# cadia-lvl/ss_asr

Measured on AMD Instinct MI355X. Metric: train-step utterances/sec on 80-dim mel, higher is better.
Workload: dtype f32; 1 GPU; BASELINE.json configs[1]: one ASRTrainer.exec iteration (GPU batch assembly from the HBM-resident corpus + engine.ASRTrainStep), ~10h synthetic Malromur-shape fbanks (8000 utts, <=800 frames, 80-dim), batch 32 per GPU, bucketed by length, LAS 256/256/128, tf_rate 0.9, Adadelta; global_batch=32, max_frames=800, parallelism=dp1, matrix_products=fp32 as 6 bf16 MFMAs on exact 3-way operand split, fp32 accumulate

## Files before the change

ss_asr_amd/csrc/common.h:

```cpp
#pragma once
#include <hip/hip_runtime.h>
#include <stdint.h>

typedef float f32x4 __attribute__((ext_vector_type(4)));

#define SSASR_OK 0
#define SSASR_EARG (-1)

#define SSASR_LAUNCH_CHECK()                         \
  do {                                               \
    hipError_t e__ = hipGetLastError();              \
    if (e__ != hipSuccess) return (int)e__;          \
  } while (0)

#define SSASR_HIP(call)                              \
  do {                                               \
    hipError_t e__ = (call);                         \
    if (e__ != hipSuccess) return (int)e__;          \
  } while (0)

struct RowMap {
  int64_t ld;
  int64_t inner;
  int64_t so;
// ... 70 lines not shown
__device__ __forceinline__ float half_max(float v) {
  v = fmaxf(v, dpp_move<0xB1>(v));
  v = fmaxf(v, dpp_move<0x4E>(v));
  v = fmaxf(v, dpp_move<0x141>(v));
  v = fmaxf(v, dpp_move<0x140>(v));
  float a;
  const float b = swap16_other(v, a);
  return fmaxf(a, b);
}
__device__ __forceinline__ float wave_sum(float v) {
  v = half_sum(v);
  const auto r = __builtin_amdgcn_permlane32_swap(__float_as_uint(v), __float_as_uint(v), false, false);
  return __uint_as_float(r[0]) + __uint_as_float(r[1]);
}
__device__ __forceinline__ float wave_max(float v) {
  v = half_max(v);
  const auto r = __builtin_amdgcn_permlane32_swap(__float_as_uint(v), __float_as_uint(v), false, false);
  return fmaxf(__uint_as_float(r[0]), __uint_as_float(r[1]));
}

struct GemmDesc {
  const float* A;
  const float* B;
  float* C;
  RowMap ma, mb, mc;
  int M, N, K;
  int ta;
  int tb;
  const float* bias1;
  const float* bias2;
  int act;
  float alpha, beta;
  int splitk;
  int batch;
  int64_t sa, sb, sc, sbias;
  int nseg;
  struct Seg {
    const float* A[2];
    const float* B[2];
    float* C[2];
    RowMap mb;
    int64_t ldc;
    int N, K;
  } seg[2];
  float* colsum[2];
  float* colsum2[2];
  int kcat;
  int64_t ska, skb;
  int tile;
};
int ssasr_launch_gemm(const GemmDesc& g, hipStream_t st);
int ssasr_launch_transpose(const float* src, float* dst, int rows, int cols, hipStream_t st);
int ssasr_launch_bptt_persistent(const float* whhT, float* gates, const float* cs, const float* dy, int64_t ys_s,
                                 int64_t ys_n, const int32_t* lens, float* gx, int32_t* sync_ws, int64_t S,
                                 int64_t N, int64_t H, int dirs, hipStream_t st, int64_t i0 = 0, int64_t i1 = 0,
                                 float* dc_state = nullptr, const float* whh_f = nullptr, const float* whh_r = nullptr,
                                 bool armed = false, const float* tsave = nullptr, void* stop_event = nullptr,
                                 const void* progress = nullptr);
struct SsasrOptions {
  int no_persistent;
  int no_fused_input;
  int bptt_halves_off;
  int bptt_reserve_kb;
  int no_persistent_decoder;
  int no_persistent_decoder_bwd;
  int delay_fwd, delay_bwd, delay_bwd_ksplit;
  int gemm_tile;
  int gemm_trace_lo, gemm_trace_hi;
  int gemm_wide;
  int gemm_bf16;
  int gemm_x6;
  int gemm_kcat;
  int no_windows;
  int bptt_one_launch;
  int wgrad_fused;
  int last_seg_pct;
  int tail_inline;
  int no_residency_check;
  int test_drop_tile;
  int test_drop_attn_slice;
  int test_drop_dec_slice;
  int attn_rph;
  int no_tsave;
};
const SsasrOptions& ssasr_options();
int64_t ssasr_resident_capacity(const void* kernel, int threads, size_t dyn_lds);
size_t ssasr_gemm_min_lds_bytes();
size_t ssasr_lds_reservation_against_gemm(const void* kernel);
bool ssasr_bptt_ksplit_ok(int64_t S, int64_t N, int64_t H, int dirs);
extern "C" int64_t ssasr_bilstm_bwd_gx_floats(int64_t S, int64_t N, int64_t H);
int ssasr_launch_colsum(const float* m, int64_t rows, int cols, int64_t ld, float* out, hipStream_t st,
                        float* out2 = nullptr);
```

ss_asr_amd/csrc/options.hip:

```cpp
#include <cstdlib>
#include <cstring>
#include <map>
#include <mutex>
#include <tuple>
#include "../../include/ssasr.h"
#include "common.h"

namespace {

SsasrOptions g_opt;
std::once_flag g_opt_once;

int env_int(const char* name, int dflt) {
  const char* v = getenv(name);
  return v ? atoi(v) : dflt;
}
int env_flag(const char* name) { return getenv(name) != nullptr; }

void init_options() {
  g_opt.no_persistent = env_flag("SSASR_NO_PERSISTENT");
  g_opt.no_fused_input = env_flag("SSASR_NO_FUSED_INPUT");
  g_opt.bptt_halves_off = env_flag("SSASR_BPTT_HALVES_OFF");
  g_opt.bptt_reserve_kb = env_flag("SSASR_BPTT_SHARED_CU") ? 0 : env_int("SSASR_BPTT_RESERVE_KB", 118);
  g_opt.no_persistent_decoder = env_flag("SSASR_NO_PERSISTENT_DECODER");
  g_opt.no_persistent_decoder_bwd = env_flag("SSASR_NO_PERSISTENT_DECODER_BWD");
  g_opt.delay_fwd = env_int("SSASR_PERSIST_DELAY_FWD", -1);
  g_opt.delay_bwd = env_int("SSASR_PERSIST_DELAY_BWD", -1);
  g_opt.delay_bwd_ksplit = g_opt.delay_bwd;
  g_opt.gemm_tile = env_int("SSASR_GEMM_TILE", 0);
  g_opt.gemm_x6 = env_int("SSASR_GEMM_X6", 1);
  g_opt.gemm_wide = env_int("SSASR_GEMM_WIDE", 1);
  g_opt.gemm_bf16 = env_int("SSASR_GEMM_BF16", 0);
  g_opt.gemm_trace_lo = g_opt.gemm_trace_hi = 0;
  g_opt.gemm_kcat = env_int("SSASR_GEMM_KCAT", 1);
  g_opt.wgrad_fused = env_int("SSASR_WGRAD_FUSED", 1);
  g_opt.bptt_one_launch = env_int("SSASR_BPTT_ONE_LAUNCH", 1);
  g_opt.no_windows = env_flag("SSASR_NO_WINDOWS");
  g_opt.last_seg_pct = env_int("SSASR_LAST_SEG_PCT", 60);
  g_opt.tail_inline = env_int("SSASR_TAIL_INLINE", 1);
  g_opt.no_residency_check = env_flag("SSASR_NO_RESIDENCY_CHECK");
  g_opt.test_drop_tile = env_int("SSASR_TEST_DROP_TILE", -1);
  g_opt.test_drop_attn_slice = env_int("SSASR_TEST_DROP_ATTN_SLICE", -1);
  g_opt.test_drop_dec_slice = env_int("SSASR_TEST_DROP_DEC_SLICE", -1);
  g_opt.attn_rph = env_int("SSASR_ATTN_RPH", 0);
  if (g_opt.attn_rph != 2 && g_opt.attn_rph != 3 && g_opt.attn_rph != 4 && g_opt.attn_rph != 6) g_opt.attn_rph = 0;
  g_opt.no_tsave = env_flag("SSASR_NO_TSAVE");
}

struct Named { const char* name; int SsasrOptions::*field; };
const Named kNames[] = {
    {"SSASR_NO_PERSISTENT", &SsasrOptions::no_persistent},
    {"SSASR_NO_FUSED_INPUT", &SsasrOptions::no_fused_input},
    {"SSASR_BPTT_HALVES_OFF", &SsasrOptions::bptt_halves_off},
    {"SSASR_BPTT_RESERVE_KB", &SsasrOptions::bptt_reserve_kb},
    {"SSASR_NO_PERSISTENT_DECODER", &SsasrOptions::no_persistent_decoder},
    {"SSASR_NO_PERSISTENT_DECODER_BWD", &SsasrOptions::no_persistent_decoder_bwd},
    {"SSASR_PERSIST_DELAY_FWD", &SsasrOptions::delay_fwd},
    {"SSASR_PERSIST_DELAY_BWD", &SsasrOptions::delay_bwd},
    {"SSASR_GEMM_TILE", &SsasrOptions::gemm_tile},
    {"SSASR_GEMM_TRACE_LO", &SsasrOptions::gemm_trace_lo},
    {"SSASR_GEMM_TRACE_HI", &SsasrOptions::gemm_trace_hi},
    {"SSASR_GEMM_X6", &SsasrOptions::gemm_x6},
    {"SSASR_GEMM_WIDE", &SsasrOptions::gemm_wide},
    {"SSASR_GEMM_BF16", &SsasrOptions::gemm_bf16},
    {"SSASR_GEMM_KCAT", &SsasrOptions::gemm_kcat},
    {"SSASR_WGRAD_FUSED", &SsasrOptions::wgrad_fused},
    {"SSASR_BPTT_ONE_LAUNCH", &SsasrOptions::bptt_one_launch},
    {"SSASR_NO_WINDOWS", &SsasrOptions::no_windows},
    {"SSASR_LAST_SEG_PCT", &SsasrOptions::last_seg_pct},
    {"SSASR_TAIL_INLINE", &SsasrOptions::tail_inline},
    {"SSASR_NO_RESIDENCY_CHECK", &SsasrOptions::no_residency_check},
    {"SSASR_TEST_DROP_TILE", &SsasrOptions::test_drop_tile},
    {"SSASR_TEST_DROP_ATTN_SLICE", &SsasrOptions::test_drop_attn_slice},
    {"SSASR_TEST_DROP_DEC_SLICE", &SsasrOptions::test_drop_dec_slice},
    {"SSASR_ATTN_RPH", &SsasrOptions::attn_rph},
    {"SSASR_NO_TSAVE", &SsasrOptions::no_tsave},
};

}

const SsasrOptions& ssasr_options() {
  std::call_once(g_opt_once, init_options);
  return g_opt;
}

extern "C" int ssasr_set_option(const char* name, int value) {
  if (!name) return SSASR_EARG;
  std::call_once(g_opt_once, init_options);
  for (const Named& n : kNames)
    if (strcmp(n.name, name) == 0) {
      g_opt.*(n.field) = value;
      if (n.field == &SsasrOptions::delay_bwd) g_opt.delay_bwd_ksplit = value;
      return SSASR_OK;
    }
  return SSASR_EARG;
}

extern "C" int ssasr_get_option(const char* name, int* value) {
  if (!name || !value) return SSASR_EARG;
  std::call_once(g_opt_once, init_options);
  for (const Named& n : kNames)
    if (strcmp(n.name, name) == 0) { *value = g_opt.*(n.field); return SSASR_OK; }
  return SSASR_EARG;
}

size_t ssasr_lds_reservation_against_gemm(const void* kernel) {
  constexpr size_t CU_LDS = 160 * 1024;
  hipFuncAttributes fa{};
  if (hipFuncGetAttributes(&fa, kernel) != hipSuccess) return 0;
  const size_t own = fa.sharedSizeBytes, gemm = ssasr_gemm_min_lds_bytes();
  if (own + gemm > CU_LDS) return 0;
  return CU_LDS - own - gemm + 1024;
}

int64_t ssasr_resident_capacity(const void* kernel, int threads, size_t dyn_lds) {
  static std::mutex mu;
  static std::map<std::tuple<const void*, int, size_t, int>, int64_t> cache;
  int dev = 0;
  if (hipGetDevice(&dev) != hipSuccess) return 0;
  std::lock_guard<std::mutex> lock(mu);
  const auto key = std::make_tuple(kernel, threads, dyn_lds, dev);
  auto it = cache.find(key);
  if (it != cache.end()) return it->second;
  int per_cu = 0, cus = 0;
  if (hipOccupancyMaxActiveBlocksPerMultiprocessor(&per_cu, kernel, threads, dyn_lds) != hipSuccess) per_cu = 0;
  if (hipDeviceGetAttribute(&cus, hipDeviceAttributeMultiprocessorCount, dev) != hipSuccess) cus = 0;
  const int64_t cap = (int64_t)per_cu * cus;
  cache[key] = cap;
  return cap;
}
```

ss_asr_amd/csrc/rnn.hip:

```cpp
#include <cstdlib>
#include <hip/hip_ext.h>
#include "../../include/ssasr.h"
#include "rnn_kernels.h"

constexpr int SSASR_MAX_SEGMENTS = 8;

int ssasr_launch_transpose(const float* src, float* dst, int rows, int cols, hipStream_t st) {
  dim3 grid((cols + 31) / 32, (rows + 31) / 32), block(32, 8);
  hipLaunchKernelGGL(transpose_kernel, grid, block, 0, st, src, dst, rows, cols);
  SSASR_LAUNCH_CHECK();
  return SSASR_OK;
}

int ssasr_launch_colsum(const float* m, int64_t rows, int cols, int64_t ld, float* out, hipStream_t st,
                        float* out2) {
  if (rows <= 0 || cols <= 0) return SSASR_OK;
  int64_t gy64 = (rows + 255) / 256;
  int gy = gy64 > 64 ? 64 : (int)gy64;
  if (gy < 1) gy = 1;
  dim3 grid((cols + 63) / 64, gy), block(256);
  if (cols % 4 == 0 && ld % 4 == 0 && aligned16(m))
    hipLaunchKernelGGL(colsum4_kernel, grid, block, 0, st, m, rows, cols, ld, out, out2);
  else
    hipLaunchKernelGGL(colsum_kernel, grid, block, 0, st, m, rows, cols, ld, out, out2);
  SSASR_LAUNCH_CHECK();
  return SSASR_OK;
}

static int persist_delay(int opt, int dflt) {
  if (opt < 0) return dflt;
  return opt > 96 ? 96 : opt;
}

static bool grid_fits(const void* kernel, int threads, size_t dyn_lds, int64_t workgroups) {
  if (ssasr_options().no_residency_check) return true;
  const int64_t cap = ssasr_resident_capacity(kernel, threads, dyn_lds);
  return cap <= 0 || workgroups <= cap;
}

constexpr int64_t PERSIST_WINDOW = 128;
static int64_t window_count(int64_t N) { return (N + PERSIST_WINDOW - 1) / PERSIST_WINDOW; }
static int64_t window_width(int64_t N, int64_t w) { return std::min<int64_t>(PERSIST_WINDOW, N - w * PERSIST_WINDOW); }

static const void* fwd_fn(int kpw, int nb, bool fuse) {
#define SSASR_FN(K, NBT) reinterpret_cast<const void*>(lstm_enc_fwd_persistent_kernel<K, NBT>)
  if (fuse) return nb == 1 ? reinterpret_cast<const void*>(lstm_enc_fwd_persistent_kernel<4, 1, 5>)
                           : reinterpret_cast<const void*>(lstm_enc_fwd_persistent_kernel<4, 2, 5>);
  return nb == 1 ? (kpw == 1 ? SSASR_FN(1, 1) : kpw == 2 ? SSASR_FN(2, 1) : kpw == 4 ? SSASR_FN(4, 1) : SSASR_FN(8, 1))
                 : (kpw == 1 ? SSASR_FN(1, 2) : kpw == 2 ? SSASR_FN(2, 2) : kpw == 4 ? SSASR_FN(4, 2) : SSASR_FN(8, 2));
#undef SSASR_FN
}
static void fwd_launch(int kpw, int nb, bool fuse, dim3 grid, hipStream_t st, const EncPersist& p) {
  const dim3 block(FWD_THREADS);
#define SSASR_L(K, NBT) hipLaunchKernelGGL((lstm_enc_fwd_persistent_kernel<K, NBT>), grid, block, 0, st, p)
  if (fuse && nb == 1) hipLaunchKernelGGL((lstm_enc_fwd_persistent_kernel<4, 1, 5>), grid, block, 0, st, p);
  else if (fuse) hipLaunchKernelGGL((lstm_enc_fwd_persistent_kernel<4, 2, 5>), grid, block, 0, st, p);
  else if (nb == 1) { if (kpw == 1) SSASR_L(1, 1); else if (kpw == 2) SSASR_L(2, 1); else if (kpw == 4) SSASR_L(4, 1); else SSASR_L(8, 1); }
  else { if (kpw == 1) SSASR_L(1, 2); else if (kpw == 2) SSASR_L(2, 2); else if (kpw == 4) SSASR_L(4, 2); else SSASR_L(8, 2); }
#undef SSASR_L
}
static int fwd_nb(int64_t Nw, int64_t H) { return (H / 4) * 2 * ((Nw + 15) / 16) <= 256 ? 1 : 2; }
static int64_t fwd_hx_floats_window(int64_t S, int64_t Nw, int64_t H) { return 2 * S * (H / 4) * ((Nw + 7) & ~(int64_t)7) * 4; }

extern "C" int64_t ssasr_bilstm_fwd_hx_floats(int64_t S, int64_t N, int64_t H) {
  if (S <= 0 || N <= 0 || H <= 0 || H % 64 != 0 || (ssasr_options().no_windows && N > PERSIST_WINDOW)) return 0;
  int64_t total = 0;
  for (int64_t w = 0; w < window_count(N); ++w) total += fwd_hx_floats_window(S, window_width(N, w), H);
  return total;
}

extern "C" int ssasr_bilstm_fwd(const float* x, int64_t xs_s, int64_t xs_n, int64_t S, int64_t N,
                                int64_t I, int64_t H, const int32_t* lens,
                                const float* w_ih_f, const float* w_hh_f, const float* b_ih_f,
                                const float* b_hh_f, const float* w_ih_r, const float* w_hh_r,
                                const float* b_ih_r, const float* b_hh_r, float* y, int64_t ys_s,
                                int64_t ys_n, float* gates, float* cs, float* hs, float* hx,
                                int32_t* sync_ws, int armed, float* tsave, void* stream) {
  const SsasrOptions& opt = ssasr_options();
  if (S <= 0 || N <= 0 || I <= 0 || H <= 0 || H % 16 != 0) return SSASR_EARG;
  if (!x || !y || !gates || (!cs && !tsave) || !hs) return SSASR_EARG;
  if (tsave && !aligned16(tsave)) return SSASR_EARG;
  hipStream_t st = (hipStream_t)stream;
  const int64_t rows = S * N;
  const float* wih[2] = {w_ih_f, w_ih_r};
  const float* whh[2] = {w_hh_f, w_hh_r};
  const float* bih[2] = {b_ih_f, b_ih_r};
  const float* bhh[2] = {b_hh_f, b_hh_r};

  auto input_projection = [&]() -> int {
    const bool paired = bih[0] && bhh[0] && bih[1] && bhh[1] && (wih[1] - wih[0]) % 4 == 0 &&
                        (bih[1] - bih[0]) == (bhh[1] - bhh[0]);
    for (int d = 0; d < (paired ? 1 : 2); ++d) {
      GemmDesc g{};
      g.A = x; g.ma = RowMap{0, N, xs_s, xs_n};
      g.B = wih[d]; g.mb = rm_dense(I);
      g.C = gates + d * rows * 4 * H; g.mc = rm_dense(4 * H);
      g.M = (int)rows; g.N = (int)(4 * H); g.K = (int)I;
      g.ta = 0; g.tb = 0; g.bias1 = bih[d]; g.bias2 = bhh[d];
      g.alpha = 1.f; g.beta = 0.f; g.splitk = 1; g.batch = 1;
      if (paired) {
        g.batch = 2; g.sa = 0; g.sb = wih[1] - wih[0]; g.sc = rows * 4 * H; g.sbias = bih[1] - bih[0];
      }
      int rc = ssasr_launch_gemm(g, st);
      if (rc) return rc;
    }
    return SSASR_OK;
  };

  if (ys_s >= (1ll << 31) || ys_n >= (1ll << 31) || rows * 4 * H >= (1ll << 40)) return SSASR_EARG;
  if (!aligned16(w_hh_f) || !aligned16(w_hh_r) || !aligned16(hs)) return SSASR_EARG;
  {
    const int kpw = (int)(H / 64);
    const int64_t nwin = window_count(N);
    bool fits = hx && sync_ws && H % 64 == 0 && (kpw == 1 || kpw == 2 || kpw == 4 || kpw == 8) &&
                aligned16(hx) && aligned16(gates) && aligned16(cs) && aligned16(y) && ys_s % 4 == 0 &&
                ys_n % 4 == 0 && !opt.no_persistent && !(opt.no_windows && nwin > 1);
    bool fuse_in = fits && kpw == 4 && I == 80 && bih[0] && bhh[0] && bih[1] && bhh[1] &&
                   aligned16(x) && aligned16(w_ih_f) && aligned16(w_ih_r) && xs_s % 4 == 0 && xs_n % 4 == 0 &&
                   !opt.no_fused_input;
    for (int64_t w = 0; w < nwin && fits; ++w) {
      const int64_t Nw = window_width(N, w), Npw = (Nw + 7) & ~(int64_t)7;
      const int nb = fwd_nb(Nw, H);
      const int64_t chunks = (Nw + 16 * nb - 1) / (16 * nb);
      if ((H / 4) * 2 * chunks > 512 || S * Npw * H * 4 >= (1ll << 31) ||
          !grid_fits(fwd_fn(kpw, nb, fuse_in), FWD_THREADS, 0, (H / 4) * 2 * chunks)) {
        fits = false; fuse_in = false;
      }
    }
    if (tsave && !fits) return SSASR_EARG;
    if (!fuse_in) {
      const int rc = input_projection();
      if (rc) return rc;
    }
    if (fits) {
      if (!armed)
        SSASR_HIP(hipMemsetD32Async((hipDeviceptr_t)hx, (int)PERSIST_SENTINEL, (size_t)ssasr_bilstm_fwd_hx_floats(S, N, H), st));
      float* hxw = hx;
      for (int64_t w = 0; w < nwin; ++w) {
        const int64_t n0 = w * PERSIST_WINDOW, Nw = window_width(N, w);
        const int nb = fwd_nb(Nw, H);
        const int64_t chunks = (Nw + 16 * nb - 1) / (16 * nb);
        EncPersist p{};
        p.tsave = tsave ? tsave + (n0 / 16) * (H / 16) * 5 * 256 : nullptr;
        p.drop_tile = opt.test_drop_tile;
        p.whh[0] = w_hh_f; p.whh[1] = w_hh_r;
        p.x = x + n0 * xs_n; p.xs_s = xs_s; p.xs_n = xs_n;
        for (int d = 0; d < 2; ++d) { p.wih[d] = wih[d]; p.bih[d] = bih[d]; p.bhh[d] = bhh[d]; }
        p.gates = gates + n0 * 4 * H; p.cs = cs ? cs + n0 * H : nullptr; p.hs = hs + n0 * H; p.hx = hxw;
        p.y = y + n0 * ys_n; p.lens = lens ? lens + n0 : nullptr;
        p.status = sync_ws + 4;
        p.delay = persist_delay(opt.delay_fwd, 24);
        p.ys_s = (int)ys_s; p.ys_n = (int)ys_n; p.S = (int)S; p.N = (int)Nw; p.H = (int)H;
        p.nt = nwin > 1 ? (int)N : 0;
        fwd_launch(kpw, nb, fuse_in, dim3((unsigned)(H / 4), 2, (unsigned)chunks), st, p);
        hxw += fwd_hx_floats_window(S, Nw, H);
      }
      SSASR_LAUNCH_CHECK();
      return SSASR_OK;
    }
  }
  if (tsave) return SSASR_EARG;
  EncFwd e{};
  e.whh[0] = w_hh_f; e.whh[1] = w_hh_r;
  e.gates = gates; e.cs = cs; e.hs = hs; e.y = y; e.lens = lens;
  e.ys_s = (int)ys_s; e.ys_n = (int)ys_n; e.S = (int)S; e.N = (int)N; e.H = (int)H;
  dim3 grid = cell_fwd_grid(H, 2, N), block(256);
  for (int64_t i = 0; i < S; ++i)
    hipLaunchKernelGGL(lstm_enc_fwd_kernel, grid, block, 0, st, e, (int)i);
  SSASR_LAUNCH_CHECK();
  return SSASR_OK;
}

static bool fwd_persistent_shape_ok(int64_t S, int64_t N, int64_t H) {
  const SsasrOptions& opt = ssasr_options();
  if (S <= 0 || N <= 0 || H <= 0 || H % 64 != 0 || opt.no_persistent || (opt.no_windows && N > PERSIST_WINDOW)) return false;
  const int kpw = (int)(H / 64);
  if (!(kpw == 1 || kpw == 2 || kpw == 4 || kpw == 8)) return false;
  for (int64_t w = 0; w < window_count(N); ++w) {
    const int64_t Nw = window_width(N, w), Npw = (Nw + 7) & ~(int64_t)7;
    const int nb = fwd_nb(Nw, H);
    const int64_t chunks = (Nw + 16 * nb - 1) / (16 * nb);
    if ((H / 4) * 2 * chunks > 512 || S * Npw * H * 4 >= (1ll << 31)) return false;
    if (!grid_fits(fwd_fn(kpw, nb, false), FWD_THREADS, 0, (H / 4) * 2 * chunks)) return false;
    if (kpw == 4 && !grid_fits(fwd_fn(kpw, nb, true), FWD_THREADS, 0, (H / 4) * 2 * chunks)) return false;
  }
  return true;
}

extern "C" int64_t ssasr_bilstm_bwd_gx_floats(int64_t S, int64_t N, int64_t H) {
  if (S <= 0 || N <= 0 || (H != 64 && H != 128 && H != 256)) return 0;
  const int64_t chunks = (N + 15) / 16;
  return 2 * chunks * BWD_RS_RING * (H / 16) * (H / 16) * 256;
}

extern "C" int64_t ssasr_bilstm_bwd_ring_floats(int64_t S, int64_t N, int64_t H, int64_t dirs) {
  if (dirs < 1 || dirs > 2 || !ssasr_bptt_ksplit_ok(S, N, H, (int)dirs)) return 0;
  return dirs * ((N + 15) / 16) * BWD_RS_RING * (H / 16) * (H / 16) * 256;
}

static const void* bptt_rs_fn(int kpw, bool halves) {
  if (kpw == 4) return reinterpret_cast<const void*>(lstm_enc_bwd_rs_kernel<1, 1>);
  if (kpw == 8) return halves ? reinterpret_cast<const void*>(lstm_enc_bwd_rs_kernel<2, 2>)
                              : reinterpret_cast<const void*>(lstm_enc_bwd_rs_kernel<2, 1>);
  return halves ? reinterpret_cast<const void*>(lstm_enc_bwd_rs_kernel<4, 2>)
                : reinterpret_cast<const void*>(lstm_enc_bwd_rs_kernel<4, 1>);
}

static int bptt_reserve_bytes(int kpw, bool halves) {
  int reserve = ssasr_options().bptt_reserve_kb * 1024;
  if (reserve) {
    const size_t need = ssasr_lds_reservation_against_gemm(bptt_rs_fn(kpw, halves));
    if ((size_t)reserve < need) reserve = (int)need;
  }
  return reserve;
}

extern "C" int64_t ssasr_bilstm_tsave_floats(int64_t S, int64_t N, int64_t H) {
  if (ssasr_options().no_tsave || !fwd_persistent_shape_ok(S, N, H) || !ssasr_bptt_ksplit_ok(S, N, H, 2)) return 0;
  return 2 * S * ((N + 15) / 16) * 16 * H * 5;
}

bool ssasr_bptt_ksplit_ok(int64_t S, int64_t N, int64_t H, int dirs) {
  const SsasrOptions& opt = ssasr_options();
  const int64_t chunks = (std::min<int64_t>(N, PERSIST_WINDOW) + 15) / 16;
  if (!(S > 0 && N > 0 && (H == 64 || H == 128 || H == 256) && (H / 16) * dirs * chunks <= 256 && !opt.no_persistent) ||
      (opt.no_windows && N > PERSIST_WINDOW))
    return false;
  const int kpw = (int)(H / 16);
  return grid_fits(bptt_rs_fn(kpw, false), 320, (size_t)bptt_reserve_bytes(kpw, false), (H / 16) * dirs * chunks);
}

struct BpttProgress { unsigned* words; int n; int bound[7]; };

static int launch_bptt_window(const float* whhT, float* gates, const float* cs, const float* dy, int64_t ys_s,
                              int64_t ys_n, const int32_t* lens, float* gx, int32_t* sync_ws, int64_t S, int64_t Nw,
                              int64_t NT, int64_t H, int dirs, hipStream_t st, int64_t i0, int64_t i1, float* dc_state,
                              const float* whh_f, const float* whh_r, const float* tsave, void* stop_event,
                              const BpttProgress* prog = nullptr) {
  const int64_t chunks = (Nw + 15) / 16;
  const int kpw = (int)(H / 16);
  const SsasrOptions& opt = ssasr_options();
  const bool ranged = i0 != 0 || i1 != S;
  EncPersistBwd p{};
  p.i0 = (int)i0; p.i1 = (int)i1; p.dc_state = dc_state;
  if (whh_f && (dirs == 1 || whh_r)) { p.whh[0] = whh_f; p.whh[1] = whh_r; }
  p.whhT = whhT; p.gates = gates; p.cs = cs; p.dy = dy; p.gx = gx; p.lens = lens; p.tsave = tsave;
  p.status = sync_ws + 4;
  p.delay = persist_delay(opt.delay_bwd_ksplit, 40);
  p.ys_s = (int)ys_s; p.ys_n = (int)ys_n; p.S = (int)S; p.N = (int)Nw; p.H = (int)H; p.nt = (int)NT;
  if (prog) {
    p.progress = prog->words; p.nbound = prog->n;
    for (int k = 0; k < prog->n; ++k) p.bound[k] = prog->bound[k];
  }
  dim3 pgrid((unsigned)(H / 16), (unsigned)dirs, (unsigned)chunks), pblock(320);
  bool halves = kpw >= 8 && (H / 16) * dirs * chunks * 2 <= 256 && i1 - i0 >= 3 && !opt.bptt_halves_off;
  int reserve = bptt_reserve_bytes(kpw, halves);
  if (halves && !grid_fits(bptt_rs_fn(kpw, true), 320, (size_t)reserve, (H / 16) * dirs * chunks * 2)) {
    halves = false;
    reserve = bptt_reserve_bytes(kpw, false);
  }
  if (!halves && !grid_fits(bptt_rs_fn(kpw, false), 320, (size_t)reserve, (H / 16) * dirs * chunks)) return SSASR_EARG;
  if (halves) pgrid.z *= 2;
  if (halves && ranged && i1 < S && i1 - i0 < 4) return SSASR_EARG;
  if (reserve) SSASR_HIP(hipFuncSetAttribute(bptt_rs_fn(kpw, halves), hipFuncAttributeMaxDynamicSharedMemorySize, reserve));
  hipEvent_t stop = (hipEvent_t)stop_event;
#define SSASR_RS_LAUNCH(TPW_, HV_) hipExtLaunchKernelGGL((lstm_enc_bwd_rs_kernel<TPW_, HV_>), pgrid, pblock, (unsigned)reserve, st, nullptr, stop, 0u, p)
  if (kpw == 4) SSASR_RS_LAUNCH(1, 1);
// ... 403 lines not shown
                                           void* events, void* stream, void* side_stream) {
  const bool armed = armed_in != 0;
  if (!dw_ih_f || !dw_hh_f || !db_f || !dw_ih_r || !dw_hh_r || !db_r || !side_stream || !events) return SSASR_EARG;
  SsasrEvents* evs = static_cast<SsasrEvents*>(events);
  hipStream_t st = (hipStream_t)stream, side = (hipStream_t)side_stream;
  float* dwih[2] = {dw_ih_f, dw_ih_r};
  float* dwhh[2] = {dw_hh_f, dw_hh_r};
  float* db[2] = {db_f, db_r};
  float* db2[2] = {db2_f, db2_r};
  int nseg = segments;
  if (nseg > SSASR_MAX_SEGMENTS) nseg = SSASR_MAX_SEGMENTS;
  if (nseg < 1 || !gx || !sync_ws || !ssasr_bptt_ksplit_ok(S, N, H, 2) || S < 32 * nseg) nseg = 1;
  int rc;
  if (nseg == 1) {
    rc = bilstm_bwd_impl(armed, tsave, dy, ys_s, ys_n, x, xs_s, xs_n, S, N, I, H, lens, w_ih_f, w_hh_f, w_ih_r, w_hh_r, gates,
                         cs, hs, dx, dxs_s, dxs_n, nullptr, nullptr, nullptr, nullptr, nullptr, nullptr, ws_whhT, ws_dc,
                         gx, sync_ws, stream);
    if (rc) return rc;
    hipEvent_t ev = evs->ev[0];
    SSASR_HIP(hipEventRecord(ev, st));
    SSASR_HIP(hipStreamWaitEvent(side, ev, 0));
    return ssasr_bilstm_wgrad(gates, x, xs_s, xs_n, hs, S, N, I, H, dw_ih_f, dw_hh_f, db_f, db2_f, dw_ih_r, dw_hh_r,
                              db_r, db2_r, 1, side_stream);
  }
  if (S <= 0 || N <= 0 || I <= 0 || H <= 0 || !dy || !x || !gates || (!cs && !tsave) || !hs || !ws_whhT || !ws_dc)
    return SSASR_EARG;
  const float* wih[2] = {w_ih_f, w_ih_r};
  if (!w_hh_f || !w_hh_r) return SSASR_EARG;
  hipEvent_t done[SSASR_MAX_SEGMENTS];
  int64_t bound[SSASR_MAX_SEGMENTS + 1];
  {
    int pct = ssasr_options().last_seg_pct;
    pct = pct < 10 ? 10 : (pct > 100 ? 100 : pct);
    const int64_t last = nseg > 1 ? std::max<int64_t>(1, (S / nseg) * pct / 100) : S;
    for (int k = 0; k < nseg; ++k) bound[k] = nseg > 1 ? k * (S - last) / (nseg - 1) : 0;
    bound[nseg] = S;
  }
  const bool one_launch = evs->can_wait && evs->progress && ssasr_options().bptt_one_launch != 0 && nseg <= 8 &&
                          window_count(N) == 1;
  unsigned wait_for[SSASR_MAX_SEGMENTS];
  unsigned* wait_word[SSASR_MAX_SEGMENTS];
  if (one_launch) {
    BpttProgress prog{};
    prog.n = nseg - 1;
    const int base = evs->next_word;
    evs->next_word = (evs->next_word + 8) % SsasrEvents::PROGRESS_WORDS;
    prog.words = evs->progress + base;
    const unsigned signals = (unsigned)((H / 16) * 2 * ((N + 15) / 16));
    for (int k = 0; k + 1 < nseg; ++k) {
      prog.bound[k] = (int)bound[k + 1];
      evs->expected[base + k] += signals;
      wait_word[k] = evs->progress + base + k;
      wait_for[k] = evs->expected[base + k];
    }
    done[nseg - 1] = evs->ev[nseg - 1];
    rc = ssasr_launch_bptt_persistent(nullptr, gates, cs, dy, ys_s, ys_n, lens, gx, sync_ws, S, N, H, 2, st, 0, S,
                                      ws_dc, w_hh_f, w_hh_r, armed, tsave, done[nseg - 1], &prog);
    if (rc) {
      for (int k = 0; k + 1 < nseg; ++k) evs->expected[base + k] -= signals;
      return rc;
    }
  } else {
    for (int k = 0; k < nseg; ++k) {
      const int64_t i0 = bound[k], i1 = bound[k + 1];
      done[k] = evs->ev[k];
      rc = ssasr_launch_bptt_persistent(nullptr, gates, cs, dy, ys_s, ys_n, lens, gx, sync_ws, S, N, H, 2, st, i0, i1,
                                        ws_dc, w_hh_f, w_hh_r, armed, tsave, done[k]);
      if (rc) return rc;
    }
  }
  const int64_t rows = S * N;
  const bool kcat = dx && ssasr_options().gemm_x6 != 0 && ssasr_options().gemm_kcat != 0 && (4 * H) % 32 == 0;
  for (int d = 0; d < (kcat ? 1 : 2) && dx; ++d) {
    GemmDesc g{};
    g.A = gates + d * rows * 4 * H; g.ma = rm_dense(4 * H);
    g.B = wih[d]; g.mb = rm_dense(I);
    g.C = dx; g.mc = RowMap{0, N, dxs_s, dxs_n};
    g.M = (int)rows; g.N = (int)I; g.K = (int)(4 * H);
    g.ta = 0; g.tb = 1; g.alpha = 1.f; g.beta = d ? 1.f : 0.f; g.splitk = 1; g.batch = 1;
    if (kcat) { g.kcat = 2; g.ska = rows * 4 * H; g.skb = wih[1] - wih[0]; }
    if ((rc = ssasr_launch_gemm(g, st))) return rc;
  }
  const bool tail_inline = !dx && ssasr_options().tail_inline != 0;
  for (int k = 0; k < nseg; ++k) {
    const int64_t i0 = bound[k], i1 = bound[k + 1];
    const bool inl = tail_inline && k == nseg - 1;
    if (inl) {
      SSASR_HIP(hipEventRecord(evs->ev[SSASR_MAX_SEGMENTS], side));
      SSASR_HIP(hipStreamWaitEvent(st, evs->ev[SSASR_MAX_SEGMENTS], 0));
    } else if (one_launch && k + 1 < nseg) {
      SSASR_HIP(hipStreamWaitValue32(side, wait_word[k], wait_for[k], hipStreamWaitValueGte, 0xffffffffu));
    } else {
      SSASR_HIP(hipStreamWaitEvent(side, done[k], 0));
    }
    if ((rc = wgrad_pair_range(S - i1, S - i0, i0, i1, gates, x, xs_s, xs_n, hs, S, N, I, H, dwih, dwhh, db, db2,
                               inl ? st : side)))
      return rc;
  }
  return SSASR_OK;
}
```

ss_asr_amd/csrc/rnn_kernels.h:

```cpp
#pragma once
#include "common.h"

#ifndef SSASR_PERSIST_PRIO
#define SSASR_PERSIST_PRIO 3
#endif
#ifndef SSASR_PTRACE
#define SSASR_PTRACE(step, slot)
#define SSASR_PTRACE_H(step, slot)
#define SSASR_PRETRY(tries)
#endif
#ifndef SSASR_STAMP
#define SSASR_STAMP(i)
#define SSASR_STAMP_DRAIN()
#else
#define SSASR_STAMP_DRAIN() asm volatile("s_waitcnt vmcnt(0)" ::: "memory")
#endif

namespace {

constexpr int MAXSEG = 3;

struct SegList {
  const float* X[MAXSEG];
  const float* W[MAXSEG];
// ... 254 lines not shown
  int S, N, H;
  const float* x;
  int64_t xs_s, xs_n;
  const float* wih[2];
  const float* bih[2];
  const float* bhh[2];
  int drop_tile;
  float* tsave;
  int nt;
};

typedef unsigned u32x4 __attribute__((ext_vector_type(4)));

__device__ __forceinline__ int64_t tsave_index(int d, int s, int chunk16, int tile16, int a, int S, int C16, int T16) {
  return (((((int64_t)d * S + s) * C16 + chunk16) * T16 + tile16) * 5 + a) * 256;
}

struct PersistRole {
  int tile, d, chunk, half, nchunk;
};
__device__ __forceinline__ PersistRole persist_role(int hv) {
  PersistRole r;
  r.nchunk = gridDim.z / hv;
  r.tile = (gridDim.x & 7) ? blockIdx.x : (blockIdx.x & 7) * (gridDim.x >> 3) + (blockIdx.x >> 3);
  r.d = blockIdx.y;
  r.chunk = blockIdx.z / hv;
  r.half = blockIdx.z % hv;
  return r;
}

__device__ __forceinline__ float4 ld4(const float* p) { return *reinterpret_cast<const float4*>(p); }

__device__ __forceinline__ int xcd_grouped_tile(int bx, int ntile) {
#ifdef SSASR_NO_TILE_GROUPING
  return bx;
#else
  return (ntile & 7) ? bx : (bx & 7) * (ntile >> 3) + (bx >> 3);
#endif
}

constexpr unsigned PERSIST_MAX_SPINS = 1u << 20;

constexpr unsigned PERSIST_SENTINEL = 0x7FC0DEADu;

enum { PK_ENC_FWD = 1, PK_ENC_BPTT = 2, PK_DEC_FWD = 4, PK_DEC_CHAIN = 5 };
__device__ __forceinline__ int persist_code(int kernel, int step) {
  const unsigned wg = blockIdx.x + gridDim.x * (blockIdx.y + gridDim.y * blockIdx.z);
  return (int)(0x40000000u | ((unsigned)kernel << 24) | ((wg & 0xfffu) << 12) | ((unsigned)step & 0xfffu));
}
__device__ __forceinline__ bool persist_give_up(unsigned tries, int* status, int code) {
  if (tries > PERSIST_MAX_SPINS) {
    if ((threadIdx.x & 63) == 0) atomicCAS(status, 0, code);
    return true;
  }
  return (tries & 255u) == 8u && __hip_atomic_load(status, __ATOMIC_RELAXED, __HIP_MEMORY_SCOPE_AGENT) != 0;
}

struct PersistPacer {
  int delay;
  int clean;
  __device__ __forceinline__ void sleep() const {
    for (int k = 0; k < delay; ++k) __builtin_amdgcn_s_sleep(1);
  }
#ifndef SSASR_PACE_UP
#define SSASR_PACE_UP 2
#endif
#ifndef SSASR_PACE_CLEAN
#define SSASR_PACE_CLEAN 2
#endif
#ifndef SSASR_PACE_DOWN
#define SSASR_PACE_DOWN 1
#endif
  __device__ __forceinline__ void update(bool missed) {
    if (missed) { delay = min(delay + SSASR_PACE_UP, 96); clean = 0; }
    else if (++clean >= SSASR_PACE_CLEAN) { delay = max(delay - SSASR_PACE_DOWN, 0); clean = 0; }
  }
};

#ifndef SSASR_FWD_HELPER_WAVE
#define SSASR_FWD_HELPER_WAVE 5
#endif
constexpr int FWD_HELPER_WAVE = SSASR_FWD_HELPER_WAVE;
constexpr int FWD_THREADS = 64 * (FWD_HELPER_WAVE + 1);
template <int KPW, int NB, int KI = 0>
__global__ __launch_bounds__(FWD_THREADS) void lstm_enc_fwd_persistent_kernel(EncPersist e) {
  __shared__ __attribute__((aligned(16))) f32x4 red[4 * NB * 64];
  __shared__ __attribute__((aligned(16))) float stage[6][16 * NB][4];
  __shared__ float addbuf[2][NB][4][64];
  __shared__ int missed;
  float* sH = &stage[5][0][0];
  const int tid = threadIdx.x, wave = tid >> 6, lane = tid & 63;
  if (wave >= 4 && wave != FWD_HELPER_WAVE) return;
  if (tid == 0) missed = 0;
  __syncthreads();
  const int r = lane & 15, q = lane >> 4;
  const PersistRole role = persist_role(1);
  const int tile = role.tile, d = role.d, chunk = role.chunk;
  const int S = e.S, N = e.N, H = e.H;
  const int n0 = chunk * 16 * NB;
  const int Np = (N + 7) & ~7;
  const int NT = e.nt > 0 ? e.nt : N;
  const int64_t rows = (int64_t)S * NT;
  float* gbase = e.gates + (int64_t)d * rows * 4 * H;
  const size_t xbytes = (size_t)S * Np * H * sizeof(float);
  float* xbase = e.hx + (int64_t)d * S * Np * H;
  const __amdgpu_buffer_rsrc_t xrs = __builtin_amdgcn_make_buffer_rsrc(xbase, 0, (int)xbytes, 0x00020000);
  const int u = 4 * tile + q;

  if (wave == FWD_HELPER_WAVE) {
    PersistPacer pacer{e.delay, 0};
    float nadd[NB][4];
    constexpr int KIN = KI > 0 ? KI : 1;
    float4 wA[KIN], xb[NB][KIN];
    float bsum[4] = {0.f, 0.f, 0.f, 0.f};
    if (KI > 0) {
      const int rowA = (r & 3) * H + 4 * tile + (r >> 2);
      const float* wp = e.wih[d] + (int64_t)rowA * (16 * KI) + 4 * q;
#pragma unroll
      for (int j = 0; j < KIN; ++j) wA[j] = ld4(wp + 16 * j);
#pragma unroll
      for (int g = 0; g < 4; ++g) bsum[g] = e.bih[d][g * H + u] + e.bhh[d][g * H + u];
    }
    auto fetch = [&](int i) {
      const int s = d ? S - 1 - i : i;
#pragma unroll
      for (int bt = 0; bt < NB; ++bt) {
        const int n = n0 + 16 * bt + r;
        if (KI > 0) {
          const float* xp = e.x + (int64_t)s * e.xs_s + (int64_t)(n < N ? n : N - 1) * e.xs_n + 4 * q;
#pragma unroll
          for (int j = 0; j < KIN; ++j) xb[bt][j] = ld4(xp + 16 * j);
        } else {
          const int64_t g0 = ((int64_t)s * NT + (n < N ? n : N - 1)) * 4 * H + u;
#pragma unroll
          for (int g = 0; g < 4; ++g) nadd[bt][g] = gbase[g0 + (int64_t)g * H];
        }
      }
    };
    auto publish = [&](int i) {
#pragma unroll
      for (int bt = 0; bt < NB; ++bt) {
        if (KI > 0) {
          f32x4 a0 = {0.f, 0.f, 0.f, 0.f}, a1 = {0.f, 0.f, 0.f, 0.f};
#pragma unroll
          for (int j = 0; j < KIN; ++j) {
            a0 = __builtin_amdgcn_mfma_f32_16x16x4f32(wA[j].x, xb[bt][j].x, a0, 0, 0, 0);
            a1 = __builtin_amdgcn_mfma_f32_16x16x4f32(wA[j].y, xb[bt][j].y, a1, 0, 0, 0);
            a0 = __builtin_amdgcn_mfma_f32_16x16x4f32(wA[j].z, xb[bt][j].z, a0, 0, 0, 0);
            a1 = __builtin_amdgcn_mfma_f32_16x16x4f32(wA[j].w, xb[bt][j].w, a1, 0, 0, 0);
          }
#pragma unroll
          for (int g = 0; g < 4; ++g) nadd[bt][g] = a0[g] + a1[g] + bsum[g];
        }
#pragma unroll
        for (int g = 0; g < 4; ++g) addbuf[i & 1][bt][g][lane] = nadd[bt][g];
      }
    };
    float* cbase = e.cs + (int64_t)d * rows * H;
    float* hbase = e.hs + (int64_t)d * rows * H;
    auto flush = [&](int i) {
      const int s = d ? S - 1 - i : i;
#pragma unroll
      for (int k = 0; k < 4; ++k) {
        const int p = lane + 64 * k;
        const int a = p / (16 * NB), col = p % (16 * NB);
        const int n = n0 + col;
        if (a < 7 && n < N) {
          const float4 v = *reinterpret_cast<const float4*>(&stage[a < 6 ? a : 5][col][0]);
          const int64_t row = (int64_t)s * NT + n;
          float* dst;
          if (a < 5 && e.tsave)
            dst = e.tsave + tsave_index(d, s, n >> 4, tile >> 2, a, S, (NT + 15) >> 4, H >> 4) + ((tile & 3) * 16 + (n & 15)) * 4;
          else
            dst = a < 4 ? gbase + row * 4 * H + (int64_t)a * H + 4 * tile
                : a == 4 ? cbase + row * H + 4 * tile
                : a == 5 ? hbase + row * H + 4 * tile
                         : e.y + (int64_t)s * e.ys_s + (int64_t)n * e.ys_n + d * H + 4 * tile;
          *reinterpret_cast<float4*>(dst) = v;
        }
      }
    };
    const int i0 = 0, i1 = S;
    if (KI == 0) {
      fetch(i0); publish(i0);
      if (i0 + 1 < i1) fetch(i0 + 1);
    }
    for (int i = i0; i < i1; ++i) {
      if (i > 0) {
        SSASR_PTRACE_H(i, 8);
        pacer.sleep();
        SSASR_PTRACE_H(i, 9);
        __syncthreads();
      }
      if (KI == 0 && i + 1 < i1) { publish(i + 1); if (i + 2 < i1) fetch(i + 2); }
      if (i > i0) flush(i - 1);
      __syncthreads();
      if (i > i0) { pacer.update(missed != 0); missed = 0; }
      __syncthreads();
    }
    flush(i1 - 1);
    return;
  }

  float4 wreg[KPW];
  {
    const int wrow = (r & 3) * H + 4 * tile + (r >> 2);
    const float* wp = e.whh[d] + (int64_t)wrow * H + 4 * q;
#pragma unroll
    for (int j = 0; j < KPW; ++j) wreg[j] = *reinterpret_cast<const float4*>(wp + (wave + 4 * j) * 16);
  }

  const int bt = wave;
  const int n = n0 + 16 * bt + r;
  const bool epi = bt < NB && n < N;
  const int i0 = 0, i1 = S;
  float cstate = 0.f;
  constexpr int KIN = KI > 0 ? KI : 1;
  float wiq[KIN], xcur[NB][KIN], xnxt[NB][KIN], xnn[NB][KIN], bsum[4] = {0.f, 0.f, 0.f, 0.f};
  auto load_x = [&](int i, float (&dst)[NB][KIN]) {
    const int s = d ? S - 1 - i : i;
#pragma unroll
    for (int t = 0; t < NB; ++t) {
      const int nn = n0 + 16 * t + r;
      const float* xp = e.x + (int64_t)s * e.xs_s + (int64_t)(nn < N ? nn : N - 1) * e.xs_n + 4 * q + wave;
#pragma unroll
      for (int j = 0; j < KIN; ++j) dst[t][j] = xp[16 * j];
    }
  };
  if (KI > 0) {
    const int rowA = (r & 3) * H + 4 * tile + (r >> 2);
    const float* wp = e.wih[d] + (int64_t)rowA * (16 * KI) + 4 * q + wave;
#pragma unroll
    for (int j = 0; j < KIN; ++j) wiq[j] = wp[16 * j];
    if (epi) {
#pragma unroll
      for (int g = 0; g < 4; ++g) bsum[g] = e.bih[d][g * H + u] + e.bhh[d][g * H + u];
    }
    load_x(i0, xcur);
    load_x(i0 + 1 < S ? i0 + 1 : i0, xnxt);
    load_x(i0 + 2 < S ? i0 + 2 : i0, xnn);
  }
  const int len = (epi && e.lens) ? e.lens[n] : 0x7fffffff;
  unsigned xo[NB];
#pragma unroll
  for (int t = 0; t < NB; ++t) {
    const int nn = n0 + 16 * t + r;
    xo[t] = (unsigned)((q * Np + (nn < N ? nn : n0)) * 16);
  }

  for (int i = i0; i < i1; ++i) {
    const int s = d ? S - 1 - i : i;
    const int sp = d ? s + 1 : s - 1;
    f32x4 acc[NB], acc2[NB];
#pragma unroll
    for (int t = 0; t < NB; ++t) { acc[t] = f32x4{0.f, 0.f, 0.f, 0.f}; acc2[t] = f32x4{0.f, 0.f, 0.f, 0.f}; }
    SSASR_PTRACE(i, 0);
    if (i > 0) {
      const unsigned sbase = (unsigned)((int64_t)sp * Np * H * 4);
      __syncthreads();
      SSASR_PTRACE(i, 2);
      float4 b[KPW][NB];
      u32x4 raw[KPW][NB];
#pragma unroll
      for (int j = 0; j < KPW; ++j) {
        const unsigned koff = (unsigned)((wave + 4 * j) * 4 * Np * 16);
#pragma unroll
        for (int t = 0; t < NB; ++t)
          raw[j][t] = __builtin_amdgcn_raw_buffer_load_b128(xrs, (int)(xo[t] + koff), (int)sbase, 16);
      }
      if (KI > 0) {
#pragma unroll
        for (int j = 0; j < KIN; ++j)
#pragma unroll
          for (int t = 0; t < NB; ++t) {
            if (j & 1) acc2[t] = __builtin_amdgcn_mfma_f32_16x16x4f32(wiq[j], xcur[t][j], acc2[t], 0, 0, 0);
            else acc[t] = __builtin_amdgcn_mfma_f32_16x16x4f32(wiq[j], xcur[t][j], acc[t], 0, 0, 0);
          }
      }
      for (unsigned tries = 0;; ++tries) {
        bool anybad = false;
#pragma unroll
        for (int j = 0; j < KPW; ++j) {
          const unsigned koff = (unsigned)((wave + 4 * j) * 4 * Np * 16);
#pragma unroll
          for (int t = 0; t < NB; ++t) {
            const bool bad = raw[j][t].x == PERSIST_SENTINEL || raw[j][t].y == PERSIST_SENTINEL ||
                             raw[j][t].z == PERSIST_SENTINEL || raw[j][t].w == PERSIST_SENTINEL;
            if (__any(bad)) {
              anybad = true;
              raw[j][t] = __builtin_amdgcn_raw_buffer_load_b128(xrs, (int)(xo[t] + koff), (int)sbase, 16);
            }
          }
        }
        if (!anybad) { SSASR_PRETRY(tries); if (tries && lane == 0) missed = 1; break; }
        if (persist_give_up(tries, e.status, persist_code(PK_ENC_FWD, i))) break;
        __builtin_amdgcn_s_sleep(2);
      }
      SSASR_PTRACE(i, 3);
#pragma unroll
      for (int j = 0; j < KPW; ++j) {
#pragma unroll
        for (int t = 0; t < NB; ++t) {
          const f32x4 f = __builtin_bit_cast(f32x4, raw[j][t]);
          b[j][t] = make_float4(f[0], f[1], f[2], f[3]);
        }
      }
      seg_group_mma<NB, KPW>(acc, acc2, wreg, b, KPW);
    } else if (KI > 0) {
#pragma unroll
      for (int j = 0; j < KIN; ++j)
#pragma unroll
        for (int t = 0; t < NB; ++t) acc[t] = __builtin_amdgcn_mfma_f32_16x16x4f32(wiq[j], xcur[t][j], acc[t], 0, 0, 0);
    }
    if (KI > 0) {
#pragma unroll
      for (int t = 0; t < NB; ++t)
#pragma unroll
        for (int j = 0; j < KIN; ++j) { xcur[t][j] = xnxt[t][j]; xnxt[t][j] = xnn[t][j]; }
      if (i + 3 < S) load_x(i + 3, xnn);
    }
#pragma unroll
    for (int t = 0; t < NB; ++t) red[(wave * NB + t) * 64 + lane] = acc[t] + acc2[t];
    SSASR_PTRACE(i, 4);
    __syncthreads();
    SSASR_PTRACE(i, 5);
    if (epi) {
      const f32x4 p = red_sum<NB>(red, bt, lane);
      float add[4];
      if (KI > 0) {
#pragma unroll
        for (int g = 0; g < 4; ++g) add[g] = bsum[g];
      } else {
        const float* ab = &addbuf[i & 1][bt][0][lane];
#pragma unroll
        for (int g = 0; g < 4; ++g) add[g] = ab[64 * g];
      }
      float gi = fast_sigmoid(p[0] + add[0]), gf = fast_sigmoid(p[1] + add[1]);
      float gg = fast_tanh(p[2] + add[2]), go = fast_sigmoid(p[3] + add[3]);
      float c = gf * cstate + gi * gg;
      float h = go * fast_tanh(c);
      if (s >= len) { gi = gf = gg = go = 0.f; c = 0.f; h = 0.f; }
      cstate = c;
      const int col = 16 * bt + r;
      stage[0][col][q] = gi;
      stage[1][col][q] = gf;
      stage[2][col][q] = gg;
      stage[3][col][q] = go;
      stage[4][col][q] = c;
      stage[5][col][q] = h;
    }
    SSASR_PTRACE(i, 6);
    __syncthreads();
    if (wave == 0) {
      if (lane < 16 * NB && n0 + lane < Np && !(tile == e.drop_tile && d == 0 && chunk == 0)) {
        const float4 hv = n0 + lane < N ? *reinterpret_cast<const float4*>(sH + lane * 4)
                                        : make_float4(0.f, 0.f, 0.f, 0.f);
        u32x4 pv = {__builtin_bit_cast(unsigned, hv.x), __builtin_bit_cast(unsigned, hv.y),
                    __builtin_bit_cast(unsigned, hv.z), __builtin_bit_cast(unsigned, hv.w)};
        __builtin_amdgcn_raw_buffer_store_b128(pv, xrs, (int)((tile * Np + n0 + lane) * 16),
                                               (int)((int64_t)s * Np * H * 4), 16);
      }
      SSASR_PTRACE(i, 7);
    }
  }
}

struct CellBwd {
  SegList sl;
  const float* add1;
  const float* add2;
  const float* dc_in;
  const float* gates;
  const float* c_prev;
  const float* c;
  float* dgates;
  float* dc_out;
  const int32_t* lens;
  int ld1, ld2;
  int s;
  int N, H;
};

struct CellBwdPair { CellBwd d[2]; };

constexpr int BWD_NB = 1;
constexpr int BWD_UN = 16;

__device__ __forceinline__ void st4(float* p, float4 v) { *reinterpret_cast<float4*>(p) = v; }

__device__ __forceinline__ void cell_bwd_body(const CellBwd& a, f32x4* red) {
  const int H = a.H, N = a.N;
  const int tile = blockIdx.x;
  const int n0 = blockIdx.z * (16 * BWD_NB);
  const int lane = threadIdx.x & 63;
  const int r = lane & 15, q = lane >> 4;

  const int bt = threadIdx.x >> 6;
// ... 571 lines not shown
```

Before: 5606 utterances/sec.

## Stage fused-input x through LDS via helper wave in persistent encoder forward

Adds an XL variant of the fused-input persistent LSTM forward kernel. The helper wave prefetches input frames from global memory into a three-slot LDS ring, and compute waves read x from LDS instead of holding three register-resident frames loaded by each wave. The aim is to cut per-wave global loads and register pressure on the serial recurrence path. The cost is extra LDS and added coordination between the helper and compute waves, and it is enabled by default. It also adds a diagnostic overlap flag, default off, that can skip the stream wait or the wgrad launch.

```diff
diff --git a/ss_asr_amd/csrc/common.h b/ss_asr_amd/csrc/common.h
--- a/ss_asr_amd/csrc/common.h
+++ b/ss_asr_amd/csrc/common.h
@@ -176,6 +176,8 @@
   int test_drop_dec_slice;
   int attn_rph;
   int no_tsave;
+  int fwd_x_lds;
+  int diag_overlap;
 };
 const SsasrOptions& ssasr_options();
 int64_t ssasr_resident_capacity(const void* kernel, int threads, size_t dyn_lds);
diff --git a/ss_asr_amd/csrc/options.hip b/ss_asr_amd/csrc/options.hip
--- a/ss_asr_amd/csrc/options.hip
+++ b/ss_asr_amd/csrc/options.hip
@@ -45,6 +45,8 @@
   g_opt.attn_rph = env_int("SSASR_ATTN_RPH", 0);
   if (g_opt.attn_rph != 2 && g_opt.attn_rph != 3 && g_opt.attn_rph != 4 && g_opt.attn_rph != 6) g_opt.attn_rph = 0;
   g_opt.no_tsave = env_flag("SSASR_NO_TSAVE");
+  g_opt.fwd_x_lds = env_int("SSASR_FWD_X_LDS", 1);
+  g_opt.diag_overlap = 0;
 }
 
 struct Named { const char* name; int SsasrOptions::*field; };
@@ -75,6 +77,8 @@
     {"SSASR_TEST_DROP_DEC_SLICE", &SsasrOptions::test_drop_dec_slice},
     {"SSASR_ATTN_RPH", &SsasrOptions::attn_rph},
     {"SSASR_NO_TSAVE", &SsasrOptions::no_tsave},
+    {"SSASR_FWD_X_LDS", &SsasrOptions::fwd_x_lds},
+    {"SSASR_DIAG_OVERLAP", &SsasrOptions::diag_overlap},
 };
 
 }
diff --git a/ss_asr_amd/csrc/rnn.hip b/ss_asr_amd/csrc/rnn.hip
--- a/ss_asr_amd/csrc/rnn.hip
+++ b/ss_asr_amd/csrc/rnn.hip
@@ -42,18 +42,22 @@
 static int64_t window_count(int64_t N) { return (N + PERSIST_WINDOW - 1) / PERSIST_WINDOW; }
 static int64_t window_width(int64_t N, int64_t w) { return std::min<int64_t>(PERSIST_WINDOW, N - w * PERSIST_WINDOW); }
 
-static const void* fwd_fn(int kpw, int nb, bool fuse) {
+static const void* fwd_fn(int kpw, int nb, bool fuse, bool xl) {
 #define SSASR_FN(K, NBT) reinterpret_cast<const void*>(lstm_enc_fwd_persistent_kernel<K, NBT>)
+  if (fuse && xl) return nb == 1 ? reinterpret_cast<const void*>(lstm_enc_fwd_persistent_kernel<4, 1, 5, 1>)
+                                 : reinterpret_cast<const void*>(lstm_enc_fwd_persistent_kernel<4, 2, 5, 1>);
   if (fuse) return nb == 1 ? reinterpret_cast<const void*>(lstm_enc_fwd_persistent_kernel<4, 1, 5>)
                            : reinterpret_cast<const void*>(lstm_enc_fwd_persistent_kernel<4, 2, 5>);
   return nb == 1 ? (kpw == 1 ? SSASR_FN(1, 1) : kpw == 2 ? SSASR_FN(2, 1) : kpw == 4 ? SSASR_FN(4, 1) : SSASR_FN(8, 1))
                  : (kpw == 1 ? SSASR_FN(1, 2) : kpw == 2 ? SSASR_FN(2, 2) : kpw == 4 ? SSASR_FN(4, 2) : SSASR_FN(8, 2));
 #undef SSASR_FN
 }
-static void fwd_launch(int kpw, int nb, bool fuse, dim3 grid, hipStream_t st, const EncPersist& p) {
+static void fwd_launch(int kpw, int nb, bool fuse, bool xl, dim3 grid, hipStream_t st, const EncPersist& p) {
   const dim3 block(FWD_THREADS);
 #define SSASR_L(K, NBT) hipLaunchKernelGGL((lstm_enc_fwd_persistent_kernel<K, NBT>), grid, block, 0, st, p)
-  if (fuse && nb == 1) hipLaunchKernelGGL((lstm_enc_fwd_persistent_kernel<4, 1, 5>), grid, block, 0, st, p);
+  if (fuse && xl && nb == 1) hipLaunchKernelGGL((lstm_enc_fwd_persistent_kernel<4, 1, 5, 1>), grid, block, 0, st, p);
+  else if (fuse && xl) hipLaunchKernelGGL((lstm_enc_fwd_persistent_kernel<4, 2, 5, 1>), grid, block, 0, st, p);
+  else if (fuse && nb == 1) hipLaunchKernelGGL((lstm_enc_fwd_persistent_kernel<4, 1, 5>), grid, block, 0, st, p);
   else if (fuse) hipLaunchKernelGGL((lstm_enc_fwd_persistent_kernel<4, 2, 5>), grid, block, 0, st, p);
   else if (nb == 1) { if (kpw == 1) SSASR_L(1, 1); else if (kpw == 2) SSASR_L(2, 1); else if (kpw == 4) SSASR_L(4, 1); else SSASR_L(8, 1); }
   else { if (kpw == 1) SSASR_L(1, 2); else if (kpw == 2) SSASR_L(2, 2); else if (kpw == 4) SSASR_L(4, 2); else SSASR_L(8, 2); }
@@ -118,12 +122,13 @@
     bool fuse_in = fits && kpw == 4 && I == 80 && bih[0] && bhh[0] && bih[1] && bhh[1] &&
                    aligned16(x) && aligned16(w_ih_f) && aligned16(w_ih_r) && xs_s % 4 == 0 && xs_n % 4 == 0 &&
                    !opt.no_fused_input;
+    const bool x_lds = fuse_in && opt.fwd_x_lds != 0;
     for (int64_t w = 0; w < nwin && fits; ++w) {
       const int64_t Nw = window_width(N, w), Npw = (Nw + 7) & ~(int64_t)7;
       const int nb = fwd_nb(Nw, H);
       const int64_t chunks = (Nw + 16 * nb - 1) / (16 * nb);
       if ((H / 4) * 2 * chunks > 512 || S * Npw * H * 4 >= (1ll << 31) ||
-          !grid_fits(fwd_fn(kpw, nb, fuse_in), FWD_THREADS, 0, (H / 4) * 2 * chunks)) {
+          !grid_fits(fwd_fn(kpw, nb, fuse_in, x_lds), FWD_THREADS, 0, (H / 4) * 2 * chunks)) {
         fits = false; fuse_in = false;
       }
     }
@@ -152,7 +157,7 @@
         p.delay = persist_delay(opt.delay_fwd, 24);
         p.ys_s = (int)ys_s; p.ys_n = (int)ys_n; p.S = (int)S; p.N = (int)Nw; p.H = (int)H;
         p.nt = nwin > 1 ? (int)N : 0;
-        fwd_launch(kpw, nb, fuse_in, dim3((unsigned)(H / 4), 2, (unsigned)chunks), st, p);
+        fwd_launch(kpw, nb, fuse_in, x_lds && fuse_in, dim3((unsigned)(H / 4), 2, (unsigned)chunks), st, p);
         hxw += fwd_hx_floats_window(S, Nw, H);
       }
       SSASR_LAUNCH_CHECK();
@@ -181,8 +186,8 @@
     const int nb = fwd_nb(Nw, H);
     const int64_t chunks = (Nw + 16 * nb - 1) / (16 * nb);
     if ((H / 4) * 2 * chunks > 512 || S * Npw * H * 4 >= (1ll << 31)) return false;
-    if (!grid_fits(fwd_fn(kpw, nb, false), FWD_THREADS, 0, (H / 4) * 2 * chunks)) return false;
-    if (kpw == 4 && !grid_fits(fwd_fn(kpw, nb, true), FWD_THREADS, 0, (H / 4) * 2 * chunks)) return false;
+    if (!grid_fits(fwd_fn(kpw, nb, false, false), FWD_THREADS, 0, (H / 4) * 2 * chunks)) return false;
+    if (kpw == 4 && !grid_fits(fwd_fn(kpw, nb, true, opt.fwd_x_lds != 0), FWD_THREADS, 0, (H / 4) * 2 * chunks)) return false;
   }
   return true;
 }
@@ -752,6 +757,7 @@
     if ((rc = ssasr_launch_gemm(g, st))) return rc;
   }
   const bool tail_inline = !dx && ssasr_options().tail_inline != 0;
+  const int diag = ssasr_options().diag_overlap;
   for (int k = 0; k < nseg; ++k) {
     const int64_t i0 = bound[k], i1 = bound[k + 1];
     const bool inl = tail_inline && k == nseg - 1;
@@ -759,10 +765,11 @@
       SSASR_HIP(hipEventRecord(evs->ev[SSASR_MAX_SEGMENTS], side));
       SSASR_HIP(hipStreamWaitEvent(st, evs->ev[SSASR_MAX_SEGMENTS], 0));
     } else if (one_launch && k + 1 < nseg) {
-      SSASR_HIP(hipStreamWaitValue32(side, wait_word[k], wait_for[k], hipStreamWaitValueGte, 0xffffffffu));
+      if (!(diag & 1)) SSASR_HIP(hipStreamWaitValue32(side, wait_word[k], wait_for[k], hipStreamWaitValueGte, 0xffffffffu));
     } else {
       SSASR_HIP(hipStreamWaitEvent(side, done[k], 0));
     }
+    if (diag & 2) continue;
     if ((rc = wgrad_pair_range(S - i1, S - i0, i0, i1, gates, x, xs_s, xs_n, hs, S, N, I, H, dwih, dwhh, db, db2,
                                inl ? st : side)))
       return rc;
diff --git a/ss_asr_amd/csrc/rnn_kernels.h b/ss_asr_amd/csrc/rnn_kernels.h
--- a/ss_asr_amd/csrc/rnn_kernels.h
+++ b/ss_asr_amd/csrc/rnn_kernels.h
@@ -360,9 +360,11 @@
 #endif
 constexpr int FWD_HELPER_WAVE = SSASR_FWD_HELPER_WAVE;
 constexpr int FWD_THREADS = 64 * (FWD_HELPER_WAVE + 1);
-template <int KPW, int NB, int KI = 0>
+template <int KPW, int NB, int KI = 0, int XL = 0>
 __global__ __launch_bounds__(FWD_THREADS) void lstm_enc_fwd_persistent_kernel(EncPersist e) {
+  static_assert(XL == 0 || KI > 0, "XL is a form of the fused input projection");
   __shared__ __attribute__((aligned(16))) f32x4 red[4 * NB * 64];
+  __shared__ float xs[XL ? 3 : 1][NB][KI > 0 ? KI : 1][4][XL ? 64 : 1];
   __shared__ __attribute__((aligned(16))) float stage[6][16 * NB][4];
   __shared__ float addbuf[2][NB][4][64];
   __shared__ int missed;
@@ -458,7 +460,36 @@
         }
       }
     };
+    float4 xq[NB][KIN];
+    auto fetch_x = [&](int i) {
+      const int s = d ? S - 1 - i : i;
+#pragma unroll
+      for (int t = 0; t < NB; ++t) {
+        const int nn = n0 + 16 * t + r;
+        const float* xp = e.x + (int64_t)s * e.xs_s + (int64_t)(nn < N ? nn : N - 1) * e.xs_n + 4 * q;
+#pragma unroll
+        for (int j = 0; j < KIN; ++j) xq[t][j] = ld4(xp + 16 * j);
+      }
+    };
+    auto put_x = [&](int slot) {
+#pragma unroll
+      for (int t = 0; t < NB; ++t)
+#pragma unroll
+        for (int j = 0; j < KIN; ++j) {
+          xs[slot][t][j][0][lane] = xq[t][j].x;
+          xs[slot][t][j][1][lane] = xq[t][j].y;
+          xs[slot][t][j][2][lane] = xq[t][j].z;
+          xs[slot][t][j][3][lane] = xq[t][j].w;
+        }
+    };
     const int i0 = 0, i1 = S;
+    if (XL) {
+      fetch_x(0); put_x(0);
+      if (1 < S) { fetch_x(1); put_x(1); }
+      if (2 < S) fetch_x(2);
+      __syncthreads();
+    }
+    int xslot = 2;
     if (KI == 0) {
       fetch(i0); publish(i0);
       if (i0 + 1 < i1) fetch(i0 + 1);
@@ -471,6 +502,11 @@
         __syncthreads();
       }
       if (KI == 0 && i + 1 < i1) { publish(i + 1); if (i + 2 < i1) fetch(i + 2); }
+      if (XL) {
+        if (i + 2 < S) put_x(xslot);
+        if (i + 3 < S) fetch_x(i + 3);
+        xslot = xslot == 2 ? 0 : xslot + 1;
+      }
       if (i > i0) flush(i - 1);
       __syncthreads();
       if (i > i0) { pacer.update(missed != 0); missed = 0; }
@@ -505,6 +541,12 @@
       for (int j = 0; j < KIN; ++j) dst[t][j] = xp[16 * j];
     }
   };
+  auto lds_x = [&](int slot) {
+#pragma unroll
+    for (int t = 0; t < NB; ++t)
+#pragma unroll
+      for (int j = 0; j < KIN; ++j) xcur[t][j] = xs[slot][t][j][wave][lane];
+  };
   if (KI > 0) {
     const int rowA = (r & 3) * H + 4 * tile + (r >> 2);
     const float* wp = e.wih[d] + (int64_t)rowA * (16 * KI) + 4 * q + wave;
@@ -514,10 +556,14 @@
 #pragma unroll
       for (int g = 0; g < 4; ++g) bsum[g] = e.bih[d][g * H + u] + e.bhh[d][g * H + u];
     }
-    load_x(i0, xcur);
-    load_x(i0 + 1 < S ? i0 + 1 : i0, xnxt);
-    load_x(i0 + 2 < S ? i0 + 2 : i0, xnn);
-  }
+    if (!XL) {
+      load_x(i0, xcur);
+      load_x(i0 + 1 < S ? i0 + 1 : i0, xnxt);
+      load_x(i0 + 2 < S ? i0 + 2 : i0, xnn);
+    }
+  }
+  if (XL) __syncthreads();
+  int xslot = 0;
   const int len = (epi && e.lens) ? e.lens[n] : 0x7fffffff;
   unsigned xo[NB];
 #pragma unroll
@@ -546,6 +592,7 @@
         for (int t = 0; t < NB; ++t)
           raw[j][t] = __builtin_amdgcn_raw_buffer_load_b128(xrs, (int)(xo[t] + koff), (int)sbase, 16);
       }
+      if (XL) lds_x(xslot);
       if (KI > 0) {
 #pragma unroll
         for (int j = 0; j < KIN; ++j)
@@ -585,12 +632,14 @@
       }
       seg_group_mma<NB, KPW>(acc, acc2, wreg, b, KPW);
     } else if (KI > 0) {
+      if (XL) lds_x(xslot);
 #pragma unroll
       for (int j = 0; j < KIN; ++j)
 #pragma unroll
         for (int t = 0; t < NB; ++t) acc[t] = __builtin_amdgcn_mfma_f32_16x16x4f32(wiq[j], xcur[t][j], acc[t], 0, 0, 0);
     }
-    if (KI > 0) {
+    if (XL) xslot = xslot == 2 ? 0 : xslot + 1;
+    if (KI > 0 && !XL) {
 #pragma unroll
       for (int t = 0; t < NB; ++t)
 #pragma unroll
```

Measured after the change: 5656 utterances/sec (median of 6 runs). About the same (+0.9%).
